# vfrantc/Bayesian-Enhancement-Model

Measured on AMD Instinct MI355X. Metric: images/sec (whole node) CG_UNet N=8 Bayesian eval @256x256, higher is better.
Workload: dtype f32

## Files before the change

### bayesian-enhancement-model_amd/csrc/gdmlp_x6.hip

```cpp
#include "bem_common.h"
#include "x6_tile.h"

namespace {

struct GdX {
    const float* x; const float* ln_w; const float* ln_b; float ln_eps;
    const u32x4* Wpi;
    const u32x4* Wpo;
    const float* bgi;
    const float* dw10;
    int C, Hd, H, W, NCH, tx;
};

struct GdPre {
    const float* y0; const float* y1; const float* on_w; const float* on_b; float on_eps;
    const u32x4* Wop;
    const float* bop; float bopmul;
};

__device__ __forceinline__ float at_byte(const float* base, uint32_t byte) {
    return *reinterpret_cast<const float*>(reinterpret_cast<const char*>(base) + byte);
}

constexpr int GD_GS = 20;

__device__ __forceinline__ float gelu_gate1(float a, float b) {
    const float t = __builtin_amdgcn_rcpf(fmaf(0.3275911f * 0.70710678118654752440f, fabsf(a), 1.f));
    float p = fmaf(1.061405429f, t, -1.453152027f);
    p = fmaf(p, t, 1.421413741f);
    p = fmaf(p, t, -0.284496736f);
    p = fmaf(p, t, 0.254829592f);
    const float e = __builtin_amdgcn_exp2f(a * a * -0.72134752044448170368f);
    const float r = fmaf(-(p * t), e, 1.f);
    const float h = 0.5f * a;
    return fmaf(h, copysignf(r, a), h) * b;
}

template <int KBM, int MTO, int WOB, bool PL2, bool PRE>
__device__ __forceinline__ void gdmlp_x6_tile(const GdX& k, const GdPre& pre, const float* __restrict__ bpo, float bomul, float* __restrict__ out) {
    constexpr int NPI = 3 * KBM, NPO = 3 * MTO;
    __shared__ __attribute__((aligned(16))) f32x2 T[16 * XT_TS];
    __shared__ __attribute__((aligned(16))) float G[128 * GD_GS];
    __shared__ __attribute__((aligned(16))) u32x4 Wis[2][NPI * 64];
    __shared__ __attribute__((aligned(16))) u32x4 Wos[WOB][NPO * 64];
    __shared__ __attribute__((aligned(16))) f32x2 Bss[2][16];
    __shared__ __attribute__((aligned(16))) f32x2 DWs[2][16 * 10];
    const int lane = threadIdx.x & 63, wave = __builtin_amdgcn_readfirstlane(threadIdx.x >> 6), kh = lane >> 5, n = lane & 31;
    const int b = blockIdx.z;
    int y0, x0;
    tile_origin(k.tx, y0, x0);
    const int L = k.H * k.W;
    const float* xb = k.x + (int64_t)b * k.C * L;

// ... 22 lines not shown
    dma_in(0, 0);
    constexpr int MTP = (8 * KBM + 15) / 16, NPW = 3 * KBM * MTP;
    static_assert(!PRE || NPW * 1024 <= (int)sizeof(T), "out_proj's rows must fit into T");
    if (PRE) {
        const uint32_t t_lds = lds_addr(T);
#pragma unroll
        for (int t = 0; t < (NPW + 3) / 4; ++t) {
            const int p = wave + 4 * t;
            if (p < NPW) glds16(pre.Wop + p * 64, voff, t_lds + p * 1024);
        }
    }

    const int oy = y0 + wave, ox = x0 + n;
    f32x16 rs[MTO];
    const bool opix = oy < k.H && ox < k.W;
    const int64_t po = (int64_t)min(oy, k.H - 1) * k.W + min(ox, k.W - 1);
    auto load_res = [&]() {
        const float* rb = (PRE ? out + (int64_t)b * k.C * L : xb) + po;
#pragma unroll
        for (int mt = 0; mt < MTO; ++mt)
#pragma unroll
            for (int r = 0; r < 16; ++r) {
                const int row = min(acc_row(r, kh, 32 * mt), k.C - 1);
                rs[mt][r] = fmaf(bpo[row], bomul, rb[(int64_t)row * L]);
            }
    };

    u32x4 xl[2][KBM][3];
    float msk[2];
    uint32_t mbit[2];
    int hpo[2];
    {
        float lnw[KBM][8], lnb[KBM][8];
        auto load_ln = [&]() {
#pragma unroll
            for (int kb = 0; kb < KBM; ++kb)
#pragma unroll
                for (int e = 0; e < 8; ++e) {
                    const int ch = 16 * kb + 8 * kh + e;
                    const float on = ch < k.C ? 1.f : 0.f;
                    lnw[kb][e] = k.ln_w[min(ch, k.C - 1)] * on;
                    lnb[kb][e] = k.ln_b[min(ch, k.C - 1)] * on;
                }
        };
        if (!PRE) load_ln();
        auto load_ln_pre = [&]() {
#pragma unroll
            for (int kb = 0; kb < KBM; ++kb) {
                const int cb = 16 * kb + 8 * kh;
                const float on = cb < k.C ? 1.f : 0.f;
                const uint32_t cbc = cb < k.C ? cb : 0;
#pragma unroll
                for (int e = 0; e < 8; ++e) {
                    lnw[kb][e] = at_byte(k.ln_w + e, 4u * cbc) * on;
                    lnb[kb][e] = at_byte(k.ln_b + e, 4u * cbc) * on;
                }
            }
        };
        float xr[2][KBM][8];
        auto load_block = [&](int i) {
            const int hp = min((wave + 4 * i) * 32 + n, XT_TS - 1);
            hpo[i] = hp;
            const int hy = hp / XT_HW, hx = hp - hy * XT_HW;
            const int gy = y0 - 1 + hy, gx = x0 - 1 + hx;
            const bool in = hp < XT_NPH && gy >= 0 && gy < k.H && gx >= 0 && gx < k.W && (wave + 4 * i) < XT_NPB;
            msk[i] = in ? 1.f : 0.f;
            mbit[i] = in ? 0xffffffffu : 0u;
            const int off = min(max(gy, 0), k.H - 1) * k.W + min(max(gx, 0), k.W - 1);
#pragma unroll
            for (int kb = 0; kb < KBM; ++kb)
#pragma unroll
                for (int e = 0; e < 8; ++e) {
                    const int ch = 16 * kb + 8 * kh + e;
                    const float v = xb[(int64_t)min(ch, k.C - 1) * L + off];
                    xr[i][kb][e] = ch < k.C ? v : 0.f;
                }
        };
        auto norm_block = [&](int i) {
            const float inv = 1.f / (float)k.C;
            float s = 0.f;
#pragma unroll
            for (int kb = 0; kb < KBM; ++kb)
#pragma unroll
                for (int e = 0; e < 8; ++e) s += xr[i][kb][e];
            s += __shfl_xor(s, 32, 64);
            const float mean = s * inv;
            float q = 0.f;
#pragma unroll
            for (int kb = 0; kb < KBM; ++kb)
#pragma unroll
                for (int e = 0; e < 8; ++e) {
                    const float d = (16 * kb + 8 * kh + e < k.C) ? xr[i][kb][e] - mean : 0.f;
                    q = fmaf(d, d, q);
                }
            q += __shfl_xor(q, 32, 64);
            const float rstd = msk[i] / sqrtf(q * inv + k.ln_eps);
#pragma unroll
            for (int kb = 0; kb < KBM; ++kb) {
                float v[8];
#pragma unroll
                for (int e = 0; e < 8; ++e) v[e] = ((xr[i][kb][e] - mean) * rstd) * lnw[kb][e] + lnb[kb][e] * msk[i];
                split8(v, xl[i][kb][0], xl[i][kb][1], xl[i][kb][2]);
            }
        };
        u32x4 yl[KBM][3];
        const float* const y0b = pre.y0 + (int64_t)b * k.C * L;
        const float* const y1b = pre.y1 + (int64_t)b * k.C * L;
        const uint32_t L4 = 4u * (uint32_t)L;
        auto tail_load = [&](int i) {
            const int hp = min((wave + 4 * i) * 32 + n, XT_TS - 1);
            hpo[i] = hp;
            const int hy = hp / XT_HW, hx = hp - hy * XT_HW;
            const int gy = y0 - 1 + hy, gx = x0 - 1 + hx;
            const bool in = hp < XT_NPH && gy >= 0 && gy < k.H && gx >= 0 && gx < k.W && (wave + 4 * i) < XT_NPB;
            msk[i] = in ? 1.f : 0.f;
            mbit[i] = in ? 0xffffffffu : 0u;
            const int off = min(max(gy, 0), k.H - 1) * k.W + min(max(gx, 0), k.W - 1);
            float ys[KBM][8];
#pragma unroll
            for (int kb = 0; kb < KBM; ++kb) {
                const int cb = 16 * kb + 8 * kh;
                const bool von = cb < k.C;
                const uint32_t a = 4u * (uint32_t)((von ? cb : 0) * L + off);
#pragma unroll
                for (int e = 0; e < 8; ++e) {
                    const float v = at_byte(y0b, a + e * L4) + at_byte(y1b, a + e * L4);
                    ys[kb][e] = von ? v : 0.f;
                }
            }
            const float inv = 1.f / (float)k.C;
            float s = 0.f;
#pragma unroll
            for (int kb = 0; kb < KBM; ++kb)
#pragma unroll
                for (int e = 0; e < 8; ++e) s += ys[kb][e];
            s += __shfl_xor(s, 32, 64);
            const float mean = s * inv;
            float q = 0.f;
#pragma unroll
            for (int kb = 0; kb < KBM; ++kb)
#pragma unroll
                for (int e = 0; e < 8; ++e) {
                    const float d = (16 * kb + 8 * kh < k.C) ? ys[kb][e] - mean : 0.f;
                    q = fmaf(d, d, q);
                }
            q += __shfl_xor(q, 32, 64);
            const float rstd = 1.f / sqrtf(q * inv + pre.on_eps);
#pragma unroll
            for (int kb = 0; kb < KBM; ++kb) {
                const int cb = 16 * kb + 8 * kh;
                const float on = cb < k.C ? 1.f : 0.f;
                const uint32_t cbc = cb < k.C ? cb : 0;
                float v[8];
#pragma unroll
                for (int e = 0; e < 8; ++e) v[e] = ((ys[kb][e] - mean) * rstd) * (at_byte(pre.on_w + e, 4u * cbc) * on) + at_byte(pre.on_b + e, 4u * cbc) * on;
                split8(v, yl[kb][0], yl[kb][1], yl[kb][2]);
            }
        };
        auto tail_gemm = [&](int i) {
            const int hp = hpo[i];
            const int hy = hp / XT_HW, hx = hp - hy * XT_HW;
            const bool ctr = mbit[i] != 0u && hy >= 1 && hy <= XT_TH && hx >= 1 && hx <= XT_TW;
            const int off = min(max(y0 - 1 + hy, 0), k.H - 1) * k.W + min(max(x0 - 1 + hx, 0), k.W - 1);
            float* const ob = out + (int64_t)b * k.C * L;
            float xv[KBM][8];
#pragma unroll
            for (int kb = 0; kb < KBM; ++kb) {
                const int cb = 16 * kb + 8 * kh;
                const uint32_t a = 4u * (uint32_t)((cb < k.C ? cb : 0) * L + off);
#pragma unroll
                for (int e = 0; e < 8; ++e) xv[kb][e] = at_byte(xb, a + e * L4);
            }
#pragma unroll
            for (int mt = 0; mt < MTP; ++mt) {
                f32x16 hi = zero16(), lo = zero16();
#pragma unroll
                for (int kb = 0; kb < KBM; ++kb) {
                    const u32x4* wp = reinterpret_cast<const u32x4*>(T) + (mt * KBM + kb) * 192 + lane;
                    const u32x4 wl[3] = {wp[0], wp[64], wp[128]};
                    mac6(wl, yl[kb], hi, lo);
                }
#pragma unroll
                for (int r = 0; r < 16; ++r) {
                    const int s = 16 * mt + r, kb = s >> 3, e = s & 7, cb = 16 * kb + 8 * kh;
                    if (s < 8 * KBM) {
                        const float v = (hi[r] + lo[r]) + at_byte(pre.bop + e, 4u * (uint32_t)(cb < k.C ? cb : 0)) * pre.bopmul + xv[kb][e];
                        xr[i][kb][e] = cb < k.C ? v : 0.f;
                    }
                }
            }
            if (ctr) {
#pragma unroll
                for (int kb = 0; kb < KBM; ++kb) {
                    const int cb = 16 * kb + 8 * kh;
                    if (cb < k.C) {
                        const uint32_t a = 4u * (uint32_t)(cb * L + off);
#pragma unroll
                        for (int e = 0; e < 8; ++e) *reinterpret_cast<float*>(reinterpret_cast<char*>(ob) + (a + e * L4)) = xr[i][kb][e];
                    }
                }
            }
        };
        if (PRE) {
            tail_load(0);
            asm volatile("s_waitcnt vmcnt(0)" ::: "memory");
            __syncthreads();
            __builtin_amdgcn_sched_barrier(0);
            tail_gemm(0);
            __builtin_amdgcn_sched_barrier(0);
            load_ln_pre();
            norm_block(0);
            __builtin_amdgcn_sched_barrier(0);
            if (wave + 4 < XT_NPB) {
// ... 3 lines not shown
                __builtin_amdgcn_sched_barrier(0);
                load_ln_pre();
                norm_block(1);
            } else {
                msk[1] = 0.f; mbit[1] = 0u; hpo[1] = XT_TS - 1;
#pragma unroll
                for (int kb = 0; kb < KBM; ++kb) xl[1][kb][0] = xl[1][kb][1] = xl[1][kb][2] = u32x4{0u, 0u, 0u, 0u};
            }
        } else if (PL2) { load_block(0); load_block(1); norm_block(0); norm_block(1); }
        else { load_block(0); norm_block(0); load_block(1); norm_block(1); }
    }

    const int wb_lds = 2 * kh * XT_HW + n;
    const int c_lo = 4 * wave;

    f32x16 oh[MTO];
#pragma unroll
    for (int mt = 0; mt < MTO; ++mt)
#pragma unroll
        for (int r = 0; r < 16; ++r) oh[mt][r] = 0.f;

    auto phase_c = [&](const u32x4* Wo) {
        const float* gp = G + (wave * 32 + n) * GD_GS + 8 * kh;
        const f32x4 ga = *reinterpret_cast<const f32x4*>(gp), gb = *reinterpret_cast<const f32x4*>(gp + 4);
        const float v[8] = {ga[0], ga[1], ga[2], ga[3], gb[0], gb[1], gb[2], gb[3]};
        u32x4 gl[3];
        split8(v, gl[0], gl[1], gl[2]);
#pragma unroll
        for (int mt = 0; mt < MTO; ++mt) {
            const u32x4* wp = Wo + mt * 192 + lane;
            const u32x4 wl[3] = {wp[0], wp[64], wp[128]};
            f32x16 lo;
#pragma unroll
            for (int r = 0; r < 16; ++r) lo[r] = 0.f;
            mac6(wl, gl, oh[mt], lo);
            oh[mt] += lo;
        }
    };

    asm volatile("s_waitcnt vmcnt(0)" ::: "memory");
    __syncthreads();

#pragma clang loop unroll(disable)
    for (int j = 0; j < k.NCH; ++j) {
        const int cur = j & 1;
        if (j + 1 < k.NCH) dma_in(j + 1, cur ^ 1);
        if (WOB == 2) dma_out(j, cur);
        const u32x4* const Wi = Wis[cur];
#pragma unroll
        for (int i = 0; i < 2; ++i) {
            if (wave + 4 * i < XT_NPB) {
                f32x16 hi, lo;
#pragma unroll
                for (int q = 0; q < 8; ++q) {
                    const f32x2 bp = Bss[cur][(q & 1) + 4 * (q >> 1) + 2 * kh];
                    lo[2 * q] = bitsf(fbits(bp[0]) & mbit[i]);
                    lo[2 * q + 1] = bitsf(fbits(bp[1]) & mbit[i]);
                    hi[2 * q] = hi[2 * q + 1] = 0.f;
                }
#pragma unroll
                for (int kb = 0; kb < KBM; ++kb) {
                    const u32x4* wp = Wi + kb * 192 + lane;
                    const u32x4 wl[3] = {wp[0], wp[64], wp[128]};
                    hi = mfma16(wl[0], xl[i][kb][0], hi);
                    lo = mfma16(wl[0], xl[i][kb][2], lo);
                    lo = mfma16(wl[2], xl[i][kb][0], lo);
                    lo = mfma16(wl[1], xl[i][kb][1], lo);
                    lo = mfma16(wl[0], xl[i][kb][1], lo);
                    lo = mfma16(wl[1], xl[i][kb][0], lo);
                }
                f32x2* tp = T + 2 * kh * XT_TS + hpo[i];
#pragma unroll
                for (int q = 0; q < 8; ++q)
                    tp[((q & 1) + 4 * (q >> 1)) * XT_TS] = f32x2{hi[2 * q] + lo[2 * q], hi[2 * q + 1] + lo[2 * q + 1]};
            }
        }
        if (j) phase_c(Wos[(j - 1) & (WOB - 1)]);
        __syncthreads();
        if (WOB == 1) dma_out(j, 0);
        {
            f32x2 g[4];
#pragma unroll
            for (int cc = 0; cc < 4; ++cc) {
                const f32x4* wv = reinterpret_cast<const f32x4*>(DWs[cur] + (c_lo + cc) * 10);
                const f32x4 w01 = wv[0], w23 = wv[1], w45 = wv[2], w67 = wv[3], w8b = wv[4];
                const f32x2 wq[9] = {{w01[0], w01[1]}, {w01[2], w01[3]}, {w23[0], w23[1]}, {w23[2], w23[3]}, {w45[0], w45[1]},
                                     {w45[2], w45[3]}, {w67[0], w67[1]}, {w67[2], w67[3]}, {w8b[0], w8b[1]}};
                const f32x2 bias = {w8b[2], w8b[3]};
                const f32x2* tp = T + (c_lo + cc) * XT_TS + wb_lds;
// ... 12 lines not shown
                        a1x = fmaf(w[0], u1[0], a1x); a1y = fmaf(w[1], u1[1], a1y);
                    }
                g[cc] = f32x2{gelu_gate1(a0x, a0y), gelu_gate1(a1x, a1y)};
            }
#pragma unroll
            for (int p = 0; p < 2; ++p)
                *reinterpret_cast<f32x4*>(G + ((2 * kh + p) * 32 + n) * GD_GS + c_lo) = f32x4{g[0][p], g[1][p], g[2][p], g[3][p]};
        }
        asm volatile("s_waitcnt vmcnt(0)" ::: "memory");
        __syncthreads();
    }
    load_res();
    phase_c(Wos[(k.NCH - 1) & (WOB - 1)]);

    if (opix) {
        float* ob = out + (int64_t)b * k.C * L + po;
#pragma unroll
        for (int mt = 0; mt < MTO; ++mt)
#pragma unroll
            for (int r = 0; r < 16; ++r) {
                const int row = acc_row(r, kh, 32 * mt);
                if (row < k.C) ob[(int64_t)row * L] = oh[mt][r] + rs[mt][r];
            }
    }
}


template <int KBM, int MTO, int WOB, bool PL2>
__global__ __launch_bounds__(256, 2) void gdmlp_x6_kernel(GdX k, const float* __restrict__ bpo, float bomul, float* __restrict__ out) {
    gdmlp_x6_tile<KBM, MTO, WOB, PL2, false>(k, GdPre{}, bpo, bomul, out);
}

template <int KBM, int MTO, int WOB>
__global__ __launch_bounds__(256, 2) void vss_back_x6_kernel(GdX k, GdPre pre, const float* __restrict__ bpo, float bomul, float* __restrict__ out) {
    gdmlp_x6_tile<KBM, MTO, WOB, false, true>(k, pre, bpo, bomul, out);
}

int gd_launch(const char* op, const float* x, const float* ln_w, const float* ln_b, float ln_eps, const float* Wp_gate, const float* bias_gate,
              const float* dw_gate10, const float* Wp_out, const float* bias_out, float* out, int B, int C, int Hd, int H, int W,
              const GdPre* pre, void* stream) {
    BEM_REQUIRE(x && ln_w && ln_b && Wp_gate && bias_gate && dw_gate10 && Wp_out && out, "%s: null tensor", op);
    BEM_REQUIRE(B >= 0 && B <= 65535 && C > 0 && C <= 80 && Hd > 0 && Hd % 16 == 0 && H > 0 && W > 0,
                "%s: needs C <= 80 and Hd %% 16 == 0 (got C = %d, Hd = %d)", op, C, Hd);
    BEM_REQUIRE((((uintptr_t)Wp_gate | (uintptr_t)Wp_out | (uintptr_t)bias_gate | (uintptr_t)dw_gate10) & 15) == 0,
                "%s: packed weights, bias pairs and depthwise parameters must be 16-byte aligned", op);
// ... 10 lines not shown
    GdX k;
    k.x = x; k.ln_w = ln_w; k.ln_b = ln_b; k.ln_eps = ln_eps;
    k.Wpi = reinterpret_cast<const u32x4*>(Wp_gate); k.Wpo = reinterpret_cast<const u32x4*>(Wp_out); k.bgi = bias_gate;
    k.dw10 = dw_gate10;
    k.C = C; k.Hd = Hd; k.H = H; k.W = W; k.NCH = Hd / 16; k.tx = cdiv(W, XT_TW);
    const float* bpop = bias_out ? bias_out : ln_w;
    const float bomul = bias_out ? 1.f : 0.f;
    dim3 grid(k.tx * cdiv(H, XT_TH), 1, B);
    hipStream_t s = (hipStream_t)stream;
    const int KB = cdiv(C, 16);
    if (pre) {
        if (KB == 1) vss_back_x6_kernel<1, 1, 2><<<grid, 256, 0, s>>>(k, *pre, bpop, bomul, out);
        else if (KB == 2) vss_back_x6_kernel<2, 1, 2><<<grid, 256, 0, s>>>(k, *pre, bpop, bomul, out);
        else vss_back_x6_kernel<3, 2, 2><<<grid, 256, 0, s>>>(k, *pre, bpop, bomul, out);
    }
    else if (KB == 1) gdmlp_x6_kernel<1, 1, 2, false><<<grid, 256, 0, s>>>(k, bpop, bomul, out);
    else if (KB == 2) gdmlp_x6_kernel<2, 1, 2, false><<<grid, 256, 0, s>>>(k, bpop, bomul, out);
    else if (KB == 3) gdmlp_x6_kernel<3, 2, 2, false><<<grid, 256, 0, s>>>(k, bpop, bomul, out);
    else if (KB == 4) gdmlp_x6_kernel<4, 2, 2, false><<<grid, 256, 0, s>>>(k, bpop, bomul, out);
    else gdmlp_x6_kernel<5, 3, 1, false><<<grid, 256, 0, s>>>(k, bpop, bomul, out);
    return bem_check_launch(op);
}

}

extern "C" int bem_gdmlp_x6_f32(const float* x, const float* ln_w, const float* ln_b, float ln_eps, const float* Wp_gate,
                                const float* bias_gate, const float* dw_gate10, const float* Wp_out,
                                const float* bias_out, float* out, int B, int C, int Hd, int H, int W, void* stream) {
    return gd_launch("gdmlp_x6", x, ln_w, ln_b, ln_eps, Wp_gate, bias_gate, dw_gate10, Wp_out, bias_out, out, B, C, Hd, H, W, nullptr, stream);
}
// ... 14 lines not shown
```

### bayesian-enhancement-model_amd/csrc/ss2d_front_x6.hip

```cpp
#include "bem_common.h"
#include "x6_tile.h"

namespace {

struct SfX {
    const float* x; const float* ln_w; const float* ln_b; float ln_eps;
    const u32x4* Wpi; const float* bi;
    const float* dww; const float* dwb;
    const u32x4* Wpx;
    float* xc; float* xd;
    int C, Mx, H, W, tx;
};

template <int KBM, int CR>
__global__ __launch_bounds__(256, 2) void ss2d_front_x6_kernel(SfX k) {
    constexpr int MTI = (CR + 31) / 32;
    constexpr int GS = CR + 4;
    __shared__ __attribute__((aligned(16))) float T[CR * XT_TS];
    __shared__ __attribute__((aligned(16))) float G[128 * GS + 8];
    __shared__ __attribute__((aligned(16))) u32x4 Wil[MTI * KBM * 3 * 64];
    __shared__ __attribute__((aligned(16))) float DWl[CR * 12];
    __shared__ float Bil[32 * MTI];
    const int lane = threadIdx.x & 63, wave = __builtin_amdgcn_readfirstlane(threadIdx.x >> 6), kh = lane >> 5, n = lane & 31;
    const int b = blockIdx.z;
    int y0, x0;
    tile_origin(k.tx, y0, x0);
    const int L = k.H * k.W;
    const float* xb = k.x + (int64_t)b * k.C * L;

    const int KB = (k.C + 15) / 16;
    {
        const uint32_t wl_lds = lds_addr(Wil), voff = 16 * lane;
#pragma unroll
        for (int t = 0; t < (MTI * KBM * 3 + 3) / 4; ++t) {
            const int p = wave + 4 * t, mt = p / (3 * KBM), kb = (p / 3) % KBM, li = p % 3;
            if (p < MTI * KBM * 3) glds16(k.Wpi + (((int64_t)mt * KB + min(kb, KB - 1)) * 3 + li) * 64, voff, wl_lds + p * 1024);
        }
    }
    for (int i = threadIdx.x; i < CR * 12; i += 256) {
        const int c = i / 12, t = i - 12 * c;
        DWl[i] = c < k.C ? (t < 9 ? k.dww[c * 9 + t] : (t == 9 && k.dwb ? k.dwb[c] : 0.f)) : 0.f;
    }
    for (int i = threadIdx.x; i < 32 * MTI; i += 256) Bil[i] = (k.bi && i < k.C) ? k.bi[i] : 0.f;
    for (int i = threadIdx.x; i < 128 * GS + 8; i += 256) G[i] = 0.f;

    u32x4 xl[2][KBM][3];
    float msk[2];
    int hpo[2];
    {
        float lnw[KBM][8], lnb[KBM][8];
#pragma unroll
        for (int kb = 0; kb < KBM; ++kb)
#pragma unroll
            for (int e = 0; e < 8; ++e) {
                const int ch = 16 * kb + 8 * kh + e;
                const float on = ch < k.C ? 1.f : 0.f;
                lnw[kb][e] = k.ln_w[min(ch, k.C - 1)] * on;
                lnb[kb][e] = k.ln_b[min(ch, k.C - 1)] * on;
            }
#pragma unroll
        for (int i = 0; i < 2; ++i) {
            const int hp = min((wave + 4 * i) * 32 + n, XT_TS - 1);
            hpo[i] = hp;
            const int hy = hp / XT_HW, hx = hp - hy * XT_HW;
            const int gy = y0 - 1 + hy, gx = x0 - 1 + hx;
            const bool in = hp < XT_NPH && gy >= 0 && gy < k.H && gx >= 0 && gx < k.W && (wave + 4 * i) < XT_NPB;
            msk[i] = in ? 1.f : 0.f;
            const int off = min(max(gy, 0), k.H - 1) * k.W + min(max(gx, 0), k.W - 1);
            float xr[KBM][8];
#pragma unroll
            for (int kb = 0; kb < KBM; ++kb)
#pragma unroll
                for (int e = 0; e < 8; ++e) {
                    const int ch = 16 * kb + 8 * kh + e;
                    const float v = xb[(int64_t)min(ch, k.C - 1) * L + off];
                    xr[kb][e] = ch < k.C ? v : 0.f;
                }
            const float inv = 1.f / (float)k.C;
            float s = 0.f;
#pragma unroll
            for (int kb = 0; kb < KBM; ++kb)
#pragma unroll
                for (int e = 0; e < 8; ++e) s += xr[kb][e];
            s += __shfl_xor(s, 32, 64);
            const float mean = s * inv;
            float q = 0.f;
#pragma unroll
            for (int kb = 0; kb < KBM; ++kb)
#pragma unroll
                for (int e = 0; e < 8; ++e) {
                    const float d = (16 * kb + 8 * kh + e < k.C) ? xr[kb][e] - mean : 0.f;
                    q = fmaf(d, d, q);
                }
            q += __shfl_xor(q, 32, 64);
            const float rstd = msk[i] / sqrtf(q * inv + k.ln_eps);
#pragma unroll
            for (int kb = 0; kb < KBM; ++kb) {
                float v[8];
#pragma unroll
                for (int e = 0; e < 8; ++e) v[e] = ((xr[kb][e] - mean) * rstd) * lnw[kb][e] + lnb[kb][e] * msk[i];
                split8(v, xl[i][kb][0], xl[i][kb][1], xl[i][kb][2]);
            }
        }
    }

    asm volatile("s_waitcnt vmcnt(0)" ::: "memory");
    __syncthreads();
#pragma unroll
    for (int i = 0; i < 2; ++i) {
        if (wave + 4 * i < XT_NPB) {
#pragma unroll
            for (int mt = 0; mt < MTI; ++mt) {
                f32x16 hi = zero16(), lo = zero16();
#pragma unroll
                for (int kb = 0; kb < KBM; ++kb) {
                    const u32x4* wp = Wil + (mt * KBM + kb) * 192 + lane;
                    u32x4 wl[3];
                    load_w3_masked(wp, kb < KB ? 0xffffffffu : 0u, wl);
                    mac6(wl, xl[i][kb], hi, lo);
                }
#pragma unroll
                for (int r = 0; r < 16; ++r) {
                    const int row = acc_row(r, kh, 32 * mt);
                    if (row < CR) T[row * XT_TS + hpo[i]] = (hi[r] + lo[r] + Bil[row]) * msk[i];
                }
            }
        }
    }
    __syncthreads();

    u32x4 wx[KBM][3];
#pragma unroll
    for (int kb = 0; kb < KBM; ++kb) {
        const u32x4* wp = k.Wpx + (int64_t)min(kb, KB - 1) * 192 + lane;
        load_w3_masked(wp, kb < KB ? 0xffffffffu : 0u, wx[kb]);
    }
    const int oy = y0 + wave, ox = x0 + n;
    const bool opix = oy < k.H && ox < k.W;
    const int64_t po = (int64_t)min(oy, k.H - 1) * k.W + min(ox, k.W - 1);
    const int chalf = k.C >> 1;
    float* xcb = k.xc + (int64_t)b * k.C * L + po;
    float* gp = G + (wave * 32 + n) * GS;
#pragma unroll 2
    for (int g0 = 0; g0 < chalf; g0 += 4) {
        f32x4 o;
#pragma unroll
        for (int j = 0; j < 4; ++j) {
            const int c = kh * chalf + g0 + j;
            const float* tp = T + c * XT_TS + wave * XT_HW + n;
            const f32x4* wv = reinterpret_cast<const f32x4*>(DWl + c * 12);
            const f32x4 w0 = wv[0], w1 = wv[1], w2 = wv[2];
            const float wq[9] = {w0[0], w0[1], w0[2], w0[3], w1[0], w1[1], w1[2], w1[3], w2[0]};
            float a = w2[1];
#pragma unroll
            for (int ty = 0; ty < 3; ++ty)
#pragma unroll
                for (int tx = 0; tx < 3; ++tx) a = fmaf(wq[3 * ty + tx], tp[ty * XT_HW + tx], a);
            o[j] = bem_silu(a);
            if (opix) xcb[(int64_t)c * L] = o[j];
        }
        *reinterpret_cast<f32x4*>(gp + kh * chalf + g0) = o;
    }

    {
        f32x16 hi = zero16(), lo = zero16();
#pragma unroll
        for (int kb = 0; kb < KBM; ++kb) {
            const float* gq = gp + 16 * kb + 8 * kh;
            const f32x4 ga = *reinterpret_cast<const f32x4*>(gq), gb = *reinterpret_cast<const f32x4*>(gq + 4);
            const float v[8] = {ga[0], ga[1], ga[2], ga[3], gb[0], gb[1], gb[2], gb[3]};
            u32x4 gl[3];
            split8(v, gl[0], gl[1], gl[2]);
            mac6(wx[kb], gl, hi, lo);
        }
        if (opix) {
            float* xdb = k.xd + (int64_t)b * k.Mx * L + po;
#pragma unroll
            for (int r = 0; r < 16; ++r) {
                const int row = acc_row(r, kh);
                if (row < k.Mx) xdb[(int64_t)row * L] = hi[r] + lo[r];
            }
        }
    }
}

}

extern "C" int bem_ss2d_front_x6_f32(const float* x, const float* ln_w, const float* ln_b, float ln_eps, const float* Wp_in, const float* bias_in,
                                     const float* dww, const float* dwb, const float* Wp_x, float* xc, float* xd, int B, int C, int Mx, int H,
                                     int W, void* stream) {
    BEM_REQUIRE(x && ln_w && ln_b && Wp_in && dww && Wp_x && xc && xd, "ss2d_front_x6: null tensor");
    BEM_REQUIRE(B >= 0 && B <= 65535 && C > 0 && C <= 48 && C % 8 == 0 && Mx > 0 && Mx <= 32 && H > 0 && W > 0,
                "ss2d_front_x6: needs C <= 48, C %% 8 == 0 and Mx <= 32 (got C = %d, Mx = %d)", C, Mx);
    BEM_REQUIRE((((uintptr_t)Wp_in | (uintptr_t)Wp_x) & 15) == 0, "ss2d_front_x6: packed weights must be 16-byte aligned");
    BEM_REQUIRE(x != xc, "ss2d_front_x6: in-place operation is not supported (halo reads)");
    BEM_REQUIRE((int64_t)C * H * W < (1ll << 31), "ss2d_front_x6: plane set too large for 32-bit offsets");
    if (B == 0) return BEM_OK;
    SfX k;
    k.x = x; k.ln_w = ln_w; k.ln_b = ln_b; k.ln_eps = ln_eps;
    k.Wpi = reinterpret_cast<const u32x4*>(Wp_in); k.bi = bias_in; k.dww = dww; k.dwb = dwb; k.Wpx = reinterpret_cast<const u32x4*>(Wp_x);
    k.xc = xc; k.xd = xd; k.C = C; k.Mx = Mx; k.H = H; k.W = W; k.tx = cdiv(W, XT_TW);
    dim3 grid(k.tx * cdiv(H, XT_TH), 1, B);
    hipStream_t s = (hipStream_t)stream;
    const int KB = cdiv(C, 16);
    if (KB == 1) ss2d_front_x6_kernel<1, 16><<<grid, 256, 0, s>>>(k);
    else if (KB == 2) ss2d_front_x6_kernel<2, 32><<<grid, 256, 0, s>>>(k);
    else if (C == 40) ss2d_front_x6_kernel<3, 40><<<grid, 256, 0, s>>>(k);
    else ss2d_front_x6_kernel<3, 48><<<grid, 256, 0, s>>>(k);
    return bem_check_launch("ss2d_front_x6");
}
```

Measured before the change: 338.6.

## Use byte-offset addressing, persistent lo accumulators and paired MFMA blocks in x6 kernels

Both x6 kernels now address global memory through precomputed byte offsets (32-bit by default, with 64-bit wide-kernel variants for huge planes). Channel clamping and masking are applied only to the last k-block, so full blocks skip the min/select work. The gdmlp kernel keeps low-part accumulators across chunks instead of re-zeroing and adding them each time, and it interleaves MFMA chains for both pixel blocks so they share weight loads. ss2d_front splits the depthwise compute from the xc stores and drops masked weight loads. The cost is higher register pressure and extra template instantiations.

```diff
diff --git a/bayesian-enhancement-model_amd/csrc/gdmlp_x6.hip b/bayesian-enhancement-model_amd/csrc/gdmlp_x6.hip
--- a/bayesian-enhancement-model_amd/csrc/gdmlp_x6.hip
+++ b/bayesian-enhancement-model_amd/csrc/gdmlp_x6.hip
@@ -18,11 +18,17 @@
     const float* bop; float bopmul;
 };
 
-__device__ __forceinline__ float at_byte(const float* base, uint32_t byte) {
+template <typename OFF>
+__device__ __forceinline__ float at_byte(const float* base, OFF byte) {
     return *reinterpret_cast<const float*>(reinterpret_cast<const char*>(base) + byte);
 }
+template <typename OFF>
+__device__ __forceinline__ void put_byte(float* base, OFF byte, float v) {
+    *reinterpret_cast<float*>(reinterpret_cast<char*>(base) + byte) = v;
+}
 
 constexpr int GD_GS = 20;
+constexpr bool GD_LO_PERSIST = true;
 
 __device__ __forceinline__ float gelu_gate1(float a, float b) {
     const float t = __builtin_amdgcn_rcpf(fmaf(0.3275911f * 0.70710678118654752440f, fabsf(a), 1.f));
@@ -36,7 +42,7 @@
     return fmaf(h, copysignf(r, a), h) * b;
 }
 
-template <int KBM, int MTO, int WOB, bool PL2, bool PRE>
+template <int KBM, int MTO, int WOB, bool PL2, bool PRE, typename OFF = uint32_t>
 __device__ __forceinline__ void gdmlp_x6_tile(const GdX& k, const GdPre& pre, const float* __restrict__ bpo, float bomul, float* __restrict__ out) {
     constexpr int NPI = 3 * KBM, NPO = 3 * MTO;
     __shared__ __attribute__((aligned(16))) f32x2 T[16 * XT_TS];
@@ -89,15 +95,21 @@
     const int oy = y0 + wave, ox = x0 + n;
     f32x16 rs[MTO];
     const bool opix = oy < k.H && ox < k.W;
-    const int64_t po = (int64_t)min(oy, k.H - 1) * k.W + min(ox, k.W - 1);
+    const OFF L4 = (OFF)4 * (OFF)L;
+    const OFF pix4 = (OFF)4 * (OFF)(min(oy, k.H - 1) * k.W + min(ox, k.W - 1));
+    const OFF po4 = pix4 + (OFF)(4 * kh) * L4, pomax = pix4 + (OFF)(k.C - 1) * L4;
     auto load_res = [&]() {
-        const float* rb = (PRE ? out + (int64_t)b * k.C * L : xb) + po;
+        const float* rb = PRE ? out + (int64_t)b * k.C * L : xb;
 #pragma unroll
         for (int mt = 0; mt < MTO; ++mt)
 #pragma unroll
             for (int r = 0; r < 16; ++r) {
-                const int row = min(acc_row(r, kh, 32 * mt), k.C - 1);
-                rs[mt][r] = fmaf(bpo[row], bomul, rb[(int64_t)row * L]);
+                const int ru = acc_row(r, 0, 32 * mt);
+                if (ru + 4 <= 16 * (KBM - 1)) rs[mt][r] = fmaf(at_byte(bpo + ru, (uint32_t)(16 * kh)), bomul, at_byte(rb, po4 + (OFF)ru * L4));
+                else if (ru < 16 * KBM) {
+                    const int row = min(ru + 4 * kh, k.C - 1);
+                    rs[mt][r] = fmaf(at_byte(bpo, (uint32_t)(4 * row)), bomul, at_byte(rb, min(po4 + (OFF)ru * L4, pomax)));
+                }
             }
     };
 
@@ -113,9 +125,15 @@
 #pragma unroll
                 for (int e = 0; e < 8; ++e) {
                     const int ch = 16 * kb + 8 * kh + e;
-                    const float on = ch < k.C ? 1.f : 0.f;
-                    lnw[kb][e] = k.ln_w[min(ch, k.C - 1)] * on;
-                    lnb[kb][e] = k.ln_b[min(ch, k.C - 1)] * on;
+                    if (kb < KBM - 1) {
+                        lnw[kb][e] = at_byte(k.ln_w + 16 * kb + e, (uint32_t)(32 * kh));
+                        lnb[kb][e] = at_byte(k.ln_b + 16 * kb + e, (uint32_t)(32 * kh));
+                    } else {
+                        const float on = ch < k.C ? 1.f : 0.f;
+                        const uint32_t c4 = 4u * (uint32_t)min(ch, k.C - 1);
+                        lnw[kb][e] = at_byte(k.ln_w, c4) * on;
+                        lnb[kb][e] = at_byte(k.ln_b, c4) * on;
+                    }
                 }
         };
         if (!PRE) load_ln();
@@ -123,8 +141,9 @@
 #pragma unroll
             for (int kb = 0; kb < KBM; ++kb) {
                 const int cb = 16 * kb + 8 * kh;
-                const float on = cb < k.C ? 1.f : 0.f;
-                const uint32_t cbc = cb < k.C ? cb : 0;
+                const bool von = kb < KBM - 1 || cb < k.C;
+                const float on = von ? 1.f : 0.f;
+                const uint32_t cbc = von ? cb : 0;
 #pragma unroll
                 for (int e = 0; e < 8; ++e) {
                     lnw[kb][e] = at_byte(k.ln_w + e, 4u * cbc) * on;
@@ -141,14 +160,17 @@
             const bool in = hp < XT_NPH && gy >= 0 && gy < k.H && gx >= 0 && gx < k.W && (wave + 4 * i) < XT_NPB;
             msk[i] = in ? 1.f : 0.f;
             mbit[i] = in ? 0xffffffffu : 0u;
-            const int off = min(max(gy, 0), k.H - 1) * k.W + min(max(gx, 0), k.W - 1);
+            const OFF off4 = (OFF)4 * (OFF)(min(max(gy, 0), k.H - 1) * k.W + min(max(gx, 0), k.W - 1));
+            const OFF a = off4 + (OFF)(8 * kh) * L4, amax = off4 + (OFF)(k.C - 1) * L4;
 #pragma unroll
             for (int kb = 0; kb < KBM; ++kb)
 #pragma unroll
                 for (int e = 0; e < 8; ++e) {
-                    const int ch = 16 * kb + 8 * kh + e;
-                    const float v = xb[(int64_t)min(ch, k.C - 1) * L + off];
-                    xr[i][kb][e] = ch < k.C ? v : 0.f;
+                    if (kb < KBM - 1) xr[i][kb][e] = at_byte(xb, a + (OFF)(16 * kb + e) * L4);
+                    else {
+                        const float v = at_byte(xb, min(a + (OFF)(16 * kb + e) * L4, amax));
+                        xr[i][kb][e] = 16 * kb + 8 * kh + e < k.C ? v : 0.f;
+                    }
                 }
         };
         auto norm_block = [&](int i) {
@@ -165,7 +187,7 @@
             for (int kb = 0; kb < KBM; ++kb)
 #pragma unroll
                 for (int e = 0; e < 8; ++e) {
-                    const float d = (16 * kb + 8 * kh + e < k.C) ? xr[i][kb][e] - mean : 0.f;
+                    const float d = (kb < KBM - 1 || 16 * kb + 8 * kh + e < k.C) ? xr[i][kb][e] - mean : 0.f;
                     q = fmaf(d, d, q);
                 }
             q += __shfl_xor(q, 32, 64);
@@ -181,7 +203,6 @@
         u32x4 yl[KBM][3];
         const float* const y0b = pre.y0 + (int64_t)b * k.C * L;
         const float* const y1b = pre.y1 + (int64_t)b * k.C * L;
-        const uint32_t L4 = 4u * (uint32_t)L;
         auto tail_load = [&](int i) {
             const int hp = min((wave + 4 * i) * 32 + n, XT_TS - 1);
             hpo[i] = hp;
@@ -195,7 +216,7 @@
 #pragma unroll
             for (int kb = 0; kb < KBM; ++kb) {
                 const int cb = 16 * kb + 8 * kh;
-                const bool von = cb < k.C;
+                const bool von = kb < KBM - 1 || cb < k.C;
                 const uint32_t a = 4u * (uint32_t)((von ? cb : 0) * L + off);
 #pragma unroll
                 for (int e = 0; e < 8; ++e) {
@@ -216,7 +237,7 @@
             for (int kb = 0; kb < KBM; ++kb)
 #pragma unroll
                 for (int e = 0; e < 8; ++e) {
-                    const float d = (16 * kb + 8 * kh < k.C) ? ys[kb][e] - mean : 0.f;
+                    const float d = (kb < KBM - 1 || 16 * kb + 8 * kh < k.C) ? ys[kb][e] - mean : 0.f;
                     q = fmaf(d, d, q);
                 }
             q += __shfl_xor(q, 32, 64);
@@ -224,8 +245,9 @@
 #pragma unroll
             for (int kb = 0; kb < KBM; ++kb) {
                 const int cb = 16 * kb + 8 * kh;
-                const float on = cb < k.C ? 1.f : 0.f;
-                const uint32_t cbc = cb < k.C ? cb : 0;
+                const bool von = kb < KBM - 1 || cb < k.C;
+                const float on = von ? 1.f : 0.f;
+                const uint32_t cbc = von ? cb : 0;
                 float v[8];
 #pragma unroll
                 for (int e = 0; e < 8; ++e) v[e] = ((ys[kb][e] - mean) * rstd) * (at_byte(pre.on_w + e, 4u * cbc) * on) + at_byte(pre.on_b + e, 4u * cbc) * on;
@@ -242,7 +264,7 @@
 #pragma unroll
             for (int kb = 0; kb < KBM; ++kb) {
                 const int cb = 16 * kb + 8 * kh;
-                const uint32_t a = 4u * (uint32_t)((cb < k.C ? cb : 0) * L + off);
+                const uint32_t a = 4u * (uint32_t)((kb < KBM - 1 || cb < k.C ? cb : 0) * L + off);
 #pragma unroll
                 for (int e = 0; e < 8; ++e) xv[kb][e] = at_byte(xb, a + e * L4);
             }
@@ -259,8 +281,9 @@
                 for (int r = 0; r < 16; ++r) {
                     const int s = 16 * mt + r, kb = s >> 3, e = s & 7, cb = 16 * kb + 8 * kh;
                     if (s < 8 * KBM) {
-                        const float v = (hi[r] + lo[r]) + at_byte(pre.bop + e, 4u * (uint32_t)(cb < k.C ? cb : 0)) * pre.bopmul + xv[kb][e];
-                        xr[i][kb][e] = cb < k.C ? v : 0.f;
+                        const bool von = kb < KBM - 1 || cb < k.C;
+                        const float v = (hi[r] + lo[r]) + at_byte(pre.bop + e, 4u * (uint32_t)(von ? cb : 0)) * pre.bopmul + xv[kb][e];
+                        xr[i][kb][e] = von ? v : 0.f;
                     }
                 }
             }
@@ -268,10 +291,10 @@
 #pragma unroll
                 for (int kb = 0; kb < KBM; ++kb) {
                     const int cb = 16 * kb + 8 * kh;
-                    if (cb < k.C) {
+                    if (kb < KBM - 1 || cb < k.C) {
                         const uint32_t a = 4u * (uint32_t)(cb * L + off);
 #pragma unroll
-                        for (int e = 0; e < 8; ++e) *reinterpret_cast<float*>(reinterpret_cast<char*>(ob) + (a + e * L4)) = xr[i][kb][e];
+                        for (int e = 0; e < 8; ++e) put_byte(ob, a + e * L4, xr[i][kb][e]);
                     }
                 }
             }
@@ -305,11 +328,16 @@
     const int wb_lds = 2 * kh * XT_HW + n;
     const int c_lo = 4 * wave;
 
-    f32x16 oh[MTO];
+    constexpr bool LOP = GD_LO_PERSIST && MTO <= 2;
+    constexpr bool A2B = KBM <= 3;
+    f32x16 oh[MTO], ol[MTO];
 #pragma unroll
     for (int mt = 0; mt < MTO; ++mt)
 #pragma unroll
-        for (int r = 0; r < 16; ++r) oh[mt][r] = 0.f;
+        for (int r = 0; r < 16; ++r) {
+            oh[mt][r] = 0.f;
+            if (LOP) ol[mt][r] = 0.f;
+        }
 
     auto phase_c = [&](const u32x4* Wo) {
         const float* gp = G + (wave * 32 + n) * GD_GS + 8 * kh;
@@ -321,11 +349,14 @@
         for (int mt = 0; mt < MTO; ++mt) {
             const u32x4* wp = Wo + mt * 192 + lane;
             const u32x4 wl[3] = {wp[0], wp[64], wp[128]};
-            f32x16 lo;
-#pragma unroll
-            for (int r = 0; r < 16; ++r) lo[r] = 0.f;
-            mac6(wl, gl, oh[mt], lo);
-            oh[mt] += lo;
+            if constexpr (LOP) mac6(wl, gl, oh[mt], ol[mt]);
+            else {
+                f32x16 lo;
+#pragma unroll
+                for (int r = 0; r < 16; ++r) lo[r] = 0.f;
+                mac6(wl, gl, oh[mt], lo);
+                oh[mt] += lo;
+            }
         }
     };
 
@@ -338,32 +369,56 @@
         if (j + 1 < k.NCH) dma_in(j + 1, cur ^ 1);
         if (WOB == 2) dma_out(j, cur);
         const u32x4* const Wi = Wis[cur];
-#pragma unroll
-        for (int i = 0; i < 2; ++i) {
-            if (wave + 4 * i < XT_NPB) {
-                f32x16 hi, lo;
-#pragma unroll
-                for (int q = 0; q < 8; ++q) {
-                    const f32x2 bp = Bss[cur][(q & 1) + 4 * (q >> 1) + 2 * kh];
-                    lo[2 * q] = bitsf(fbits(bp[0]) & mbit[i]);
-                    lo[2 * q + 1] = bitsf(fbits(bp[1]) & mbit[i]);
-                    hi[2 * q] = hi[2 * q + 1] = 0.f;
-                }
-#pragma unroll
-                for (int kb = 0; kb < KBM; ++kb) {
-                    const u32x4* wp = Wi + kb * 192 + lane;
-                    const u32x4 wl[3] = {wp[0], wp[64], wp[128]};
-                    hi = mfma16(wl[0], xl[i][kb][0], hi);
-                    lo = mfma16(wl[0], xl[i][kb][2], lo);
-                    lo = mfma16(wl[2], xl[i][kb][0], lo);
-                    lo = mfma16(wl[1], xl[i][kb][1], lo);
-                    lo = mfma16(wl[0], xl[i][kb][1], lo);
-                    lo = mfma16(wl[1], xl[i][kb][0], lo);
-                }
-                f32x2* tp = T + 2 * kh * XT_TS + hpo[i];
-#pragma unroll
-                for (int q = 0; q < 8; ++q)
-                    tp[((q & 1) + 4 * (q >> 1)) * XT_TS] = f32x2{hi[2 * q] + lo[2 * q], hi[2 * q + 1] + lo[2 * q + 1]};
+        auto a_init = [&](int i, f32x16& hi, f32x16& lo) {
+#pragma unroll
+            for (int q = 0; q < 8; ++q) {
+                const f32x2 bp = Bss[cur][(q & 1) + 4 * (q >> 1) + 2 * kh];
+                lo[2 * q] = bitsf(fbits(bp[0]) & mbit[i]);
+                lo[2 * q + 1] = bitsf(fbits(bp[1]) & mbit[i]);
+                hi[2 * q] = hi[2 * q + 1] = 0.f;
+            }
+        };
+        auto a_mac = [&](const u32x4 (&wl)[3], const u32x4 (&x)[3], f32x16& hi, f32x16& lo) {
+            hi = mfma16(wl[0], x[0], hi);
+            lo = mfma16(wl[0], x[2], lo);
+            lo = mfma16(wl[2], x[0], lo);
+            lo = mfma16(wl[1], x[1], lo);
+            lo = mfma16(wl[0], x[1], lo);
+            lo = mfma16(wl[1], x[0], lo);
+        };
+        auto a_store = [&](int i, const f32x16& hi, const f32x16& lo) {
+            f32x2* tp = T + 2 * kh * XT_TS + hpo[i];
+#pragma unroll
+            for (int q = 0; q < 8; ++q)
+                tp[((q & 1) + 4 * (q >> 1)) * XT_TS] = f32x2{hi[2 * q] + lo[2 * q], hi[2 * q + 1] + lo[2 * q + 1]};
+        };
+        if (A2B && wave + 4 < XT_NPB) {
+            f32x16 hi0, lo0, hi1, lo1;
+            a_init(0, hi0, lo0);
+            a_init(1, hi1, lo1);
+#pragma unroll
+            for (int kb = 0; kb < KBM; ++kb) {
+                const u32x4* wp = Wi + kb * 192 + lane;
+                const u32x4 wl[3] = {wp[0], wp[64], wp[128]};
+                a_mac(wl, xl[0][kb], hi0, lo0);
+                a_mac(wl, xl[1][kb], hi1, lo1);
+            }
+            a_store(0, hi0, lo0);
+            a_store(1, hi1, lo1);
+        } else {
+#pragma unroll
+            for (int i = 0; i < 2; ++i) {
+                if (wave + 4 * i < XT_NPB) {
+                    f32x16 hi, lo;
+                    a_init(i, hi, lo);
+#pragma unroll
+                    for (int kb = 0; kb < KBM; ++kb) {
+                        const u32x4* wp = Wi + kb * 192 + lane;
+                        const u32x4 wl[3] = {wp[0], wp[64], wp[128]};
+                        a_mac(wl, xl[i][kb], hi, lo);
+                    }
+                    a_store(i, hi, lo);
+                }
             }
         }
         if (j) phase_c(Wos[(j - 1) & (WOB - 1)]);
@@ -406,13 +461,17 @@
     phase_c(Wos[(k.NCH - 1) & (WOB - 1)]);
 
     if (opix) {
-        float* ob = out + (int64_t)b * k.C * L + po;
+        float* ob = out + (int64_t)b * k.C * L;
 #pragma unroll
         for (int mt = 0; mt < MTO; ++mt)
 #pragma unroll
             for (int r = 0; r < 16; ++r) {
-                const int row = acc_row(r, kh, 32 * mt);
-                if (row < k.C) ob[(int64_t)row * L] = oh[mt][r] + rs[mt][r];
+                const int ru = acc_row(r, 0, 32 * mt);
+                const float v = (LOP ? oh[mt][r] + ol[mt][r] : oh[mt][r]) + rs[mt][r];
+                if (ru + 4 <= 16 * (KBM - 1)) put_byte(ob, po4 + (OFF)ru * L4, v);
+                else if (ru < 16 * KBM) {
+                    if (ru + 4 * kh < k.C) put_byte(ob, po4 + (OFF)ru * L4, v);
+                }
             }
     }
 }
@@ -421,6 +480,11 @@
 template <int KBM, int MTO, int WOB, bool PL2>
 __global__ __launch_bounds__(256, 2) void gdmlp_x6_kernel(GdX k, const float* __restrict__ bpo, float bomul, float* __restrict__ out) {
     gdmlp_x6_tile<KBM, MTO, WOB, PL2, false>(k, GdPre{}, bpo, bomul, out);
+}
+
+template <int KBM, int MTO, int WOB>
+__global__ __launch_bounds__(256, 1) void gdmlp_x6_wide_kernel(GdX k, const float* __restrict__ bpo, float bomul, float* __restrict__ out) {
+    gdmlp_x6_tile<KBM, MTO, WOB, false, false, uint64_t>(k, GdPre{}, bpo, bomul, out);
 }
 
 template <int KBM, int MTO, int WOB>
@@ -461,6 +525,13 @@
         else if (KB == 2) vss_back_x6_kernel<2, 1, 2><<<grid, 256, 0, s>>>(k, *pre, bpop, bomul, out);
         else vss_back_x6_kernel<3, 2, 2><<<grid, 256, 0, s>>>(k, *pre, bpop, bomul, out);
     }
+    else if ((int64_t)C * H * W >= (1ll << 30)) {
+        if (KB == 1) gdmlp_x6_wide_kernel<1, 1, 2><<<grid, 256, 0, s>>>(k, bpop, bomul, out);
+        else if (KB == 2) gdmlp_x6_wide_kernel<2, 1, 2><<<grid, 256, 0, s>>>(k, bpop, bomul, out);
+        else if (KB == 3) gdmlp_x6_wide_kernel<3, 2, 2><<<grid, 256, 0, s>>>(k, bpop, bomul, out);
+        else if (KB == 4) gdmlp_x6_wide_kernel<4, 2, 2><<<grid, 256, 0, s>>>(k, bpop, bomul, out);
+        else gdmlp_x6_wide_kernel<5, 3, 1><<<grid, 256, 0, s>>>(k, bpop, bomul, out);
+    }
     else if (KB == 1) gdmlp_x6_kernel<1, 1, 2, false><<<grid, 256, 0, s>>>(k, bpop, bomul, out);
     else if (KB == 2) gdmlp_x6_kernel<2, 1, 2, false><<<grid, 256, 0, s>>>(k, bpop, bomul, out);
     else if (KB == 3) gdmlp_x6_kernel<3, 2, 2, false><<<grid, 256, 0, s>>>(k, bpop, bomul, out);
diff --git a/bayesian-enhancement-model_amd/csrc/ss2d_front_x6.hip b/bayesian-enhancement-model_amd/csrc/ss2d_front_x6.hip
--- a/bayesian-enhancement-model_amd/csrc/ss2d_front_x6.hip
+++ b/bayesian-enhancement-model_amd/csrc/ss2d_front_x6.hip
@@ -12,10 +12,28 @@
     int C, Mx, H, W, tx;
 };
 
-template <int KBM, int CR>
-__global__ __launch_bounds__(256, 2) void ss2d_front_x6_kernel(SfX k) {
+template <typename OFF>
+__device__ __forceinline__ float at_byte(const float* base, OFF byte) {
+    return *reinterpret_cast<const float*>(reinterpret_cast<const char*>(base) + byte);
+}
+template <typename OFF>
+__device__ __forceinline__ void put_byte(float* base, OFF byte, float v) {
+    *reinterpret_cast<float*>(reinterpret_cast<char*>(base) + byte) = v;
+}
+
+constexpr bool SF_SILU_RCP = true;
+
+__device__ __forceinline__ float silu_rcp(float x) {
+    const float d = 1.f + bem_fexp(fminf(-x, 80.f));
+    const float r = __builtin_amdgcn_rcpf(d);
+    return x * fmaf(fmaf(-d, r, 1.f), r, r);
+}
+
+template <int KBM, int CR, int CC, typename OFF>
+__device__ __forceinline__ void ss2d_front_x6_tile(const SfX& k) {
     constexpr int MTI = (CR + 31) / 32;
     constexpr int GS = CR + 4;
+    constexpr int NG = CR / 8;
     __shared__ __attribute__((aligned(16))) float T[CR * XT_TS];
     __shared__ __attribute__((aligned(16))) float G[128 * GS + 8];
     __shared__ __attribute__((aligned(16))) u32x4 Wil[MTI * KBM * 3 * 64];
@@ -23,26 +41,35 @@
     __shared__ float Bil[32 * MTI];
     const int lane = threadIdx.x & 63, wave = __builtin_amdgcn_readfirstlane(threadIdx.x >> 6), kh = lane >> 5, n = lane & 31;
     const int b = blockIdx.z;
+    const int C = CC ? CC : k.C;
     int y0, x0;
     tile_origin(k.tx, y0, x0);
     const int L = k.H * k.W;
-    const float* xb = k.x + (int64_t)b * k.C * L;
-
-    const int KB = (k.C + 15) / 16;
+    const OFF L4 = (OFF)4 * (OFF)L;
+    const float* xb = k.x + (int64_t)b * C * L;
+
     {
         const uint32_t wl_lds = lds_addr(Wil), voff = 16 * lane;
 #pragma unroll
         for (int t = 0; t < (MTI * KBM * 3 + 3) / 4; ++t) {
-            const int p = wave + 4 * t, mt = p / (3 * KBM), kb = (p / 3) % KBM, li = p % 3;
-            if (p < MTI * KBM * 3) glds16(k.Wpi + (((int64_t)mt * KB + min(kb, KB - 1)) * 3 + li) * 64, voff, wl_lds + p * 1024);
-        }
-    }
-    for (int i = threadIdx.x; i < CR * 12; i += 256) {
-        const int c = i / 12, t = i - 12 * c;
-        DWl[i] = c < k.C ? (t < 9 ? k.dww[c * 9 + t] : (t == 9 && k.dwb ? k.dwb[c] : 0.f)) : 0.f;
-    }
-    for (int i = threadIdx.x; i < 32 * MTI; i += 256) Bil[i] = (k.bi && i < k.C) ? k.bi[i] : 0.f;
-    for (int i = threadIdx.x; i < 128 * GS + 8; i += 256) G[i] = 0.f;
+            const int p = wave + 4 * t;
+            if (p < MTI * KBM * 3) glds16(k.Wpi + (int64_t)p * 64, voff, wl_lds + p * 1024);
+        }
+    }
+    if (threadIdx.x < CR) {
+        const int c = threadIdx.x, cc = min(c, C - 1);
+        const float on = c < C ? 1.f : 0.f;
+        float w[12];
+#pragma unroll
+        for (int t = 0; t < 9; ++t) w[t] = k.dww[cc * 9 + t] * on;
+        w[9] = k.dwb ? k.dwb[cc] * on : 0.f;
+        w[10] = w[11] = 0.f;
+        f32x4* dp = reinterpret_cast<f32x4*>(DWl + 12 * c);
+#pragma unroll
+        for (int q = 0; q < 3; ++q) dp[q] = f32x4{w[4 * q], w[4 * q + 1], w[4 * q + 2], w[4 * q + 3]};
+    }
+    if (threadIdx.x < 32 * MTI) Bil[threadIdx.x] = (k.bi && (int)threadIdx.x < C) ? k.bi[min((int)threadIdx.x, C - 1)] : 0.f;
+    if (threadIdx.x < 8) G[128 * GS + threadIdx.x] = 0.f;
 
     u32x4 xl[2][KBM][3];
     float msk[2];
@@ -50,14 +77,16 @@
     {
         float lnw[KBM][8], lnb[KBM][8];
 #pragma unroll
-        for (int kb = 0; kb < KBM; ++kb)
+        for (int kb = 0; kb < KBM; ++kb) {
+            const bool von = kb < KBM - 1 || 16 * kb + 8 * kh < C;
+            const uint32_t c4 = von ? 32u * kh : 0u;
 #pragma unroll
             for (int e = 0; e < 8; ++e) {
-                const int ch = 16 * kb + 8 * kh + e;
-                const float on = ch < k.C ? 1.f : 0.f;
-                lnw[kb][e] = k.ln_w[min(ch, k.C - 1)] * on;
-                lnb[kb][e] = k.ln_b[min(ch, k.C - 1)] * on;
-            }
+                const float w = at_byte(k.ln_w + 16 * kb + e, c4), bb = at_byte(k.ln_b + 16 * kb + e, c4);
+                lnw[kb][e] = kb < KBM - 1 ? w : (von ? w : 0.f);
+                lnb[kb][e] = kb < KBM - 1 ? bb : (von ? bb : 0.f);
+            }
+        }
 #pragma unroll
         for (int i = 0; i < 2; ++i) {
             const int hp = min((wave + 4 * i) * 32 + n, XT_TS - 1);
@@ -66,17 +95,20 @@
             const int gy = y0 - 1 + hy, gx = x0 - 1 + hx;
             const bool in = hp < XT_NPH && gy >= 0 && gy < k.H && gx >= 0 && gx < k.W && (wave + 4 * i) < XT_NPB;
             msk[i] = in ? 1.f : 0.f;
-            const int off = min(max(gy, 0), k.H - 1) * k.W + min(max(gx, 0), k.W - 1);
+            const OFF off4 = (OFF)4 * (OFF)(min(max(gy, 0), k.H - 1) * k.W + min(max(gx, 0), k.W - 1));
+            const OFF a = off4 + (kh ? (OFF)8 * L4 : (OFF)0);
             float xr[KBM][8];
 #pragma unroll
-            for (int kb = 0; kb < KBM; ++kb)
+            for (int kb = 0; kb < KBM; ++kb) {
+                const bool von = kb < KBM - 1 || 16 * kb + 8 * kh < C;
+                const OFF ak = kb < KBM - 1 ? a : (von ? a : off4 - (OFF)(16 * kb) * L4);
 #pragma unroll
                 for (int e = 0; e < 8; ++e) {
-                    const int ch = 16 * kb + 8 * kh + e;
-                    const float v = xb[(int64_t)min(ch, k.C - 1) * L + off];
-                    xr[kb][e] = ch < k.C ? v : 0.f;
-                }
-            const float inv = 1.f / (float)k.C;
+                    const float v = at_byte(xb, ak + (OFF)(16 * kb + e) * L4);
+                    xr[kb][e] = kb < KBM - 1 ? v : (von ? v : 0.f);
+                }
+            }
+            const float inv = 1.f / (float)C;
             float s = 0.f;
 #pragma unroll
             for (int kb = 0; kb < KBM; ++kb)
@@ -89,7 +121,7 @@
             for (int kb = 0; kb < KBM; ++kb)
 #pragma unroll
                 for (int e = 0; e < 8; ++e) {
-                    const float d = (16 * kb + 8 * kh + e < k.C) ? xr[kb][e] - mean : 0.f;
+                    const float d = (kb < KBM - 1 || 16 * kb + 8 * kh < C) ? xr[kb][e] - mean : 0.f;
                     q = fmaf(d, d, q);
                 }
             q += __shfl_xor(q, 32, 64);
@@ -115,14 +147,13 @@
 #pragma unroll
                 for (int kb = 0; kb < KBM; ++kb) {
                     const u32x4* wp = Wil + (mt * KBM + kb) * 192 + lane;
-                    u32x4 wl[3];
-                    load_w3_masked(wp, kb < KB ? 0xffffffffu : 0u, wl);
+                    const u32x4 wl[3] = {wp[0], wp[64], wp[128]};
                     mac6(wl, xl[i][kb], hi, lo);
                 }
 #pragma unroll
                 for (int r = 0; r < 16; ++r) {
                     const int row = acc_row(r, kh, 32 * mt);
-                    if (row < CR) T[row * XT_TS + hpo[i]] = (hi[r] + lo[r] + Bil[row]) * msk[i];
+                    if (32 * mt + 8 * (r >> 2) < CR) T[row * XT_TS + hpo[i]] = (hi[r] + lo[r] + Bil[row]) * msk[i];
                 }
             }
         }
@@ -132,41 +163,52 @@
     u32x4 wx[KBM][3];
 #pragma unroll
     for (int kb = 0; kb < KBM; ++kb) {
-        const u32x4* wp = k.Wpx + (int64_t)min(kb, KB - 1) * 192 + lane;
-        load_w3_masked(wp, kb < KB ? 0xffffffffu : 0u, wx[kb]);
+        const u32x4* wp = k.Wpx + kb * 192 + lane;
+#pragma unroll
+        for (int li = 0; li < 3; ++li) wx[kb][li] = wp[64 * li];
     }
     const int oy = y0 + wave, ox = x0 + n;
     const bool opix = oy < k.H && ox < k.W;
-    const int64_t po = (int64_t)min(oy, k.H - 1) * k.W + min(ox, k.W - 1);
-    const int chalf = k.C >> 1;
-    float* xcb = k.xc + (int64_t)b * k.C * L + po;
+    const OFF pix4 = (OFF)4 * (OFF)(min(oy, k.H - 1) * k.W + min(ox, k.W - 1));
+    const int chalf = C >> 1;
     float* gp = G + (wave * 32 + n) * GS;
-#pragma unroll 2
-    for (int g0 = 0; g0 < chalf; g0 += 4) {
-        f32x4 o;
-#pragma unroll
-        for (int j = 0; j < 4; ++j) {
-            const int c = kh * chalf + g0 + j;
-            const float* tp = T + c * XT_TS + wave * XT_HW + n;
-            const f32x4* wv = reinterpret_cast<const f32x4*>(DWl + c * 12);
-            const f32x4 w0 = wv[0], w1 = wv[1], w2 = wv[2];
-            const float wq[9] = {w0[0], w0[1], w0[2], w0[3], w1[0], w1[1], w1[2], w1[3], w2[0]};
-            float a = w2[1];
-#pragma unroll
-            for (int ty = 0; ty < 3; ++ty)
-#pragma unroll
-                for (int tx = 0; tx < 3; ++tx) a = fmaf(wq[3 * ty + tx], tp[ty * XT_HW + tx], a);
-            o[j] = bem_silu(a);
-            if (opix) xcb[(int64_t)c * L] = o[j];
-        }
-        *reinterpret_cast<f32x4*>(gp + kh * chalf + g0) = o;
+    f32x4 o[NG];
+#pragma unroll
+    for (int g = 0; g < NG; ++g) {
+        if (4 * g < chalf) {
+#pragma unroll
+            for (int j = 0; j < 4; ++j) {
+                const int c = kh * chalf + 4 * g + j;
+                const float* tp = T + c * XT_TS + wave * XT_HW + n;
+                const f32x4* wv = reinterpret_cast<const f32x4*>(DWl + c * 12);
+                const f32x4 w0 = wv[0], w1 = wv[1], w2 = wv[2];
+                const float wq[9] = {w0[0], w0[1], w0[2], w0[3], w1[0], w1[1], w1[2], w1[3], w2[0]};
+                float a = w2[1];
+#pragma unroll
+                for (int ty = 0; ty < 3; ++ty)
+#pragma unroll
+                    for (int tx = 0; tx < 3; ++tx) a = fmaf(wq[3 * ty + tx], tp[ty * XT_HW + tx], a);
+                o[g][j] = SF_SILU_RCP ? silu_rcp(a) : bem_silu(a);
+            }
+            *reinterpret_cast<f32x4*>(gp + kh * chalf + 4 * g) = o[g];
+        }
+    }
+    if (opix) {
+        float* xcb = k.xc + (int64_t)b * C * L;
+        const OFF pc = pix4 + (kh ? (OFF)chalf * L4 : (OFF)0);
+#pragma unroll
+        for (int g = 0; g < NG; ++g)
+            if (4 * g < chalf) {
+#pragma unroll
+                for (int j = 0; j < 4; ++j) put_byte(xcb, pc + (OFF)(4 * g + j) * L4, o[g][j]);
+            }
     }
 
     {
         f32x16 hi = zero16(), lo = zero16();
 #pragma unroll
         for (int kb = 0; kb < KBM; ++kb) {
-            const float* gq = gp + 16 * kb + 8 * kh;
+            const float* gq = (kb < KBM - 1 || 16 * kb + 8 * kh < C) ? gp + 16 * kb + 8 * kh : G + 128 * GS;
             const f32x4 ga = *reinterpret_cast<const f32x4*>(gq), gb = *reinterpret_cast<const f32x4*>(gq + 4);
             const float v[8] = {ga[0], ga[1], ga[2], ga[3], gb[0], gb[1], gb[2], gb[3]};
             u32x4 gl[3];
@@ -174,14 +216,25 @@
             mac6(wx[kb], gl, hi, lo);
         }
         if (opix) {
-            float* xdb = k.xd + (int64_t)b * k.Mx * L + po;
+            float* xdb = k.xd + (int64_t)b * k.Mx * L;
+            const OFF pd = pix4 + (kh ? (OFF)4 * L4 : (OFF)0);
 #pragma unroll
             for (int r = 0; r < 16; ++r) {
-                const int row = acc_row(r, kh);
-                if (row < k.Mx) xdb[(int64_t)row * L] = hi[r] + lo[r];
-            }
-        }
-    }
+                const int ru = acc_row(r, 0);
+                if (ru + 4 * kh < k.Mx) put_byte(xdb, pd + (OFF)ru * L4, hi[r] + lo[r]);
+            }
+        }
+    }
+}
+
+template <int KBM, int CR>
+__global__ __launch_bounds__(256, 2) void ss2d_front_x6_kernel(SfX k) {
+    ss2d_front_x6_tile<KBM, CR, (KBM == 3 ? CR : 0), uint32_t>(k);
+}
+
+template <int KBM, int CR>
+__global__ __launch_bounds__(256, 1) void ss2d_front_x6_wide_kernel(SfX k) {
+    ss2d_front_x6_tile<KBM, CR, (KBM == 3 ? CR : 0), uint64_t>(k);
 }
 
 }
@@ -194,7 +247,7 @@
                 "ss2d_front_x6: needs C <= 48, C %% 8 == 0 and Mx <= 32 (got C = %d, Mx = %d)", C, Mx);
     BEM_REQUIRE((((uintptr_t)Wp_in | (uintptr_t)Wp_x) & 15) == 0, "ss2d_front_x6: packed weights must be 16-byte aligned");
     BEM_REQUIRE(x != xc, "ss2d_front_x6: in-place operation is not supported (halo reads)");
-    BEM_REQUIRE((int64_t)C * H * W < (1ll << 31), "ss2d_front_x6: plane set too large for 32-bit offsets");
+    BEM_REQUIRE((int64_t)max(C, Mx) * H * W < (1ll << 31), "ss2d_front_x6: plane set too large for 32-bit offsets");
     if (B == 0) return BEM_OK;
     SfX k;
     k.x = x; k.ln_w = ln_w; k.ln_b = ln_b; k.ln_eps = ln_eps;
@@ -203,7 +256,13 @@
     dim3 grid(k.tx * cdiv(H, XT_TH), 1, B);
     hipStream_t s = (hipStream_t)stream;
     const int KB = cdiv(C, 16);
-    if (KB == 1) ss2d_front_x6_kernel<1, 16><<<grid, 256, 0, s>>>(k);
+    if ((int64_t)max(C, Mx) * H * W >= (1ll << 30)) {
+        if (KB == 1) ss2d_front_x6_wide_kernel<1, 16><<<grid, 256, 0, s>>>(k);
+        else if (KB == 2) ss2d_front_x6_wide_kernel<2, 32><<<grid, 256, 0, s>>>(k);
+        else if (C == 40) ss2d_front_x6_wide_kernel<3, 40><<<grid, 256, 0, s>>>(k);
+        else ss2d_front_x6_wide_kernel<3, 48><<<grid, 256, 0, s>>>(k);
+    }
+    else if (KB == 1) ss2d_front_x6_kernel<1, 16><<<grid, 256, 0, s>>>(k);
     else if (KB == 2) ss2d_front_x6_kernel<2, 32><<<grid, 256, 0, s>>>(k);
     else if (C == 40) ss2d_front_x6_kernel<3, 40><<<grid, 256, 0, s>>>(k);
     else ss2d_front_x6_kernel<3, 48><<<grid, 256, 0, s>>>(k);
```

New measurement: 352.7, median of 6. 4.1% higher.
